# leagrieder/MultiMeditron

Measured on AMD Instinct MI355X. Metric: image-text samples/sec/node fwd+bwd, Llama-3.1-8B+ViT-L/14 bf16, higher is better.
Workload: dtype bf16; 1 GPU; llama31_8b_vitl14_s2048_b4; per_gpu_batch=4, global_batch=4, seq_len=2048, training_mode=FULL, parallelism=dp1

## Files before the change

include/mm_hip.h:

```cpp
#ifndef MM_HIP_H
#define MM_HIP_H

#include <stdint.h>

#ifdef __cplusplus
extern "C" {
#endif

typedef enum { MM_BF16 = 0, MM_F32 = 1 } mm_dtype;

enum { MM_OK = 0, MM_ERR_ARG = -1, MM_ERR_ALIGN = -2, MM_ERR_UNSUPPORTED = -3, MM_ERR_LAUNCH = -4 };

enum {
  MM_GEMM_NT = 0,
  MM_GEMM_NN = 1,
  MM_GEMM_TN = 2
};

enum {
  MM_EPI_BIAS = 1,
  MM_EPI_GELU_ERF = 2,
  MM_EPI_QUICK_GELU = 4,
  MM_EPI_RESIDUAL = 8,
  MM_EPI_ACCUMULATE = 16,
// ... 23 lines not shown

int mm_splice_build_map(const int64_t* batch_idx, const int64_t* token_range, int n_mod, int S, int T,
                        int32_t* src_map, void* stream);
int mm_embed_splice_fwd(int dtype, const void* emb, int64_t vocab, int H, const int64_t* ids, const void* proj,
                        const int32_t* src_map, int T, void* out, void* stream);
int mm_embed_sort_sizes(int T, int H, int64_t* order_elems, int64_t* scratch_floats);
int mm_embed_sort(const int64_t* ids, const int32_t* src_map, int T, int64_t vocab, int32_t* key_ws, int32_t* order,
                  int32_t* skey, void* stream);
int mm_embed_splice_bwd(int dtype, const void* dE, int H, const int64_t* ids, const int32_t* src_map, int T,
                        const int64_t* batch_idx, const int64_t* token_range, int n_mod, int S, void* dproj,
                        void* demb, int64_t vocab, const int32_t* order, const int32_t* skey, float* scratch,
                        int accumulate, void* stream);

int mm_patchify(int dtype, const float* pixels, int n, int himg, int wimg, int ps, int kpad, void* patches, void* stream);
int mm_vit_embed_fwd(int dtype, const void* patch_out, const void* cls, const void* pos, int n, int P, int D,
                     void* x, void* stream);
int mm_vit_embed_bwd(int dtype, const void* dx, int n, int P, int D, void* dpatch_out, void* dcls, void* dpos,
                     int accumulate, void* stream);
int mm_bcast_add(int dtype, const void* x, const void* b, int n, int64_t L, void* y, void* stream);
int mm_head_pad(int dtype, const void* src, int64_t rows, int nheads, int d, int dpad, void* dst, int inverse, void* stream);
int mm_drop_cls_fwd(int dtype, const void* src, int n, int P, int D, void* dst, void* stream);
int mm_drop_cls_bwd(int dtype, const void* ddst, int n, int P, int D, void* dsrc, void* stream);
int mm_rows_select(int dtype, const void* src, int64_t ld_src, const int* map, int n_src, int n_dst, int D, void* dst,
                   int64_t ld_dst, void* stream);

int mm_rmsnorm_fwd(int dtype, const void* x, const void* w, int M, int H, float eps, void* y, float* rstd, void* stream);
int mm_rmsnorm_bwd(int dtype, const void* dy, const void* x, const void* w, const float* rstd, int M, int H,
                   void* dx, float* dw_partial, const void* dres, void* stream);
int mm_layernorm_fwd(int dtype, const void* x, const void* w, const void* b, int M, int H, float eps, void* y,
                     float* mean, float* rstd, void* stream);
int mm_layernorm_bwd(int dtype, const void* dy, const void* x, const void* w, const float* mean, const float* rstd,
                     int M, int H, void* dx, float* dw_partial, float* db_partial, const void* dres, void* stream);
int mm_norm_bwd_blocks(int M);
int mm_reduce_partials(int dtype, const float* partial, int nblk, int H, void* out, int accumulate, void* stream);
int mm_reduce_partials2(int dtype, const float* partial0, const float* partial1, int nblk, int H, void* out0, void* out1, int accumulate0,
                        int accumulate1, void* stream);

int mm_rope_table(const int64_t* position_ids, const float* inv_freq, int T, int half, int round_bf16, float* cos_t,
                  float* sin_t, void* stream);
int mm_rope_apply(int dtype, void* x, int T, int nheads, int D, int ld, const float* cos_t, const float* sin_t,
                  int inverse, void* stream);

int mm_attn_fwd(int dtype, const void* q, const void* k, const void* v, int B, int Sq, int Skv, int Hq, int Hkv, int D,
                int64_t q_sb, int64_t q_ss, int64_t q_sh, int64_t k_sb, int64_t k_ss, int64_t k_sh, int64_t v_sb,
                int64_t v_ss, int64_t v_sh, const int64_t* key_mask, int causal, float scale, void* out, float* lse,
                void* stream);
int mm_attn_bwd(int dtype, const void* q, const void* k, const void* v, const void* out, const void* dout, const float* lse,
                int B, int Sq, int Skv, int Hq, int Hkv, int D, int64_t q_sb, int64_t q_ss, int64_t q_sh, int64_t k_sb,
                int64_t k_ss, int64_t k_sh, int64_t v_sb, int64_t v_ss, int64_t v_sh, const int64_t* key_mask, int causal,
                float scale, void* dq, void* dk, void* dv, float* delta, void* stream);

int mm_rope_append(int dtype, void* x, int T, int Hq, int Hkv, int D, int ld, const float* cos_t, const float* sin_t,
                   void* kdst, void* vdst, int64_t dstride, void* stream);

int mm_qk_norm_rope_fwd(int dtype, const void* x, int ld_in, int T, int Hq, int Hkv, int D, const void* w_q, const void* w_k, float eps,
                        const float* cos_t, const float* sin_t, void* out, int ld_out, float* rstd, void* stream);
int mm_qk_norm_bwd_blocks(int T);
int mm_qk_norm_rope_bwd(int dtype, const void* dqk, int ld_dqk, const void* x, int ld_x, int T, int Hq, int Hkv, int D, const void* w_q,
                        const void* w_k, const float* rstd, const float* cos_t, const float* sin_t, void* dx, int ld_dx, float* dwq_partial,
                        float* dwk_partial, void* stream);
int mm_qk_norm_rope_append(int dtype, void* x, int T, int Hq, int Hkv, int D, int ld, const void* w_q, const void* w_k, float eps,
                           const float* cos_t, const float* sin_t, void* kdst, void* vdst, int64_t dstride, void* stream);

int mm_decode_gateup_swiglu(int dtype, int M, int I, int K, const void* X, int ldx, const void* Wgu, int ldw, void* ACT, int ldact,
                            const void* in_norm_w, float eps, void* stream);
int mm_decode_qkv_rope_append(int dtype, int M, int Hq, int Hkv, int D, int K, const void* X, int ldx, const void* W, int ldw,
// ... 89 lines not shown
```

multimeditron_amd/csrc/mm_attn.hip:

```cpp
#include <string.h>

#include "mm_common.h"

namespace {

struct AttnArgs {
  const void *q, *k, *v;
  int B, Sq, Skv, Hq, Hkv;
  int64_t q_sb, q_ss, q_sh, k_sb, k_ss, k_sh, v_sb, v_ss, v_sh;
  const int64_t* kmask;
  int causal;
  float scale;
  void* out;
  float* lse;
  const void* dout;
  const float* delta;
  void *dq, *dk, *dv;
  int diag;
  int prio;
};

constexpr float LOG2E = 1.4426950408889634f;
constexpr float LN2 = 0.6931471805599453f;

template <int D> __device__ __forceinline__ int v_swz(int row) {
  if constexpr (D == 128) return (row & 3) << 1;
  else return ((row >> 1) & 1) << 1;
}

template <int D, int ROWS>
struct KcStage {
  static constexpr int NI = ROWS * (D / 8) / 256;
  u32x4 r[NI];
  __device__ __forceinline__ void load(const bf16* base, int64_t row_stride, int row0, int nrows_valid) {
    const int l = threadIdx.x & 63, w = threadIdx.x >> 6;
    constexpr int HALVES = D / 64;
#pragma unroll
    for (int i = 0; i < NI; ++i) {
      const int u = w * NI + i;
      const int rg = u / HALVES, dh = u % HALVES;
      const int row = rg * 8 + (l & 7), dc = dh * 8 + (l >> 3);
      u32x4 v = {0u, 0u, 0u, 0u};
      if (row0 + row < nrows_valid) v = *(const u32x4*)(base + (int64_t)(row0 + row) * row_stride + dc * 8);
      r[i] = v;
    }
  }
  __device__ __forceinline__ void store(char* tile) const {
    const int l = threadIdx.x & 63, w = threadIdx.x >> 6;
    constexpr int HALVES = D / 64;
#pragma unroll
// ... 193 lines not shown
    for (int db = 0; db < NDB; ++db)
#pragma unroll
      for (int rg = 0; rg < 4; ++rg) {
        bf16x4 o;
#pragma unroll
        for (int e = 0; e < 4; ++e) o[e] = (bf16)(o_acc[db][rg * 4 + e] * inv);
        *(bf16x4*)(orow + db * 32 + 8 * rg + 4 * h) = o;
      }
    if (h == 0) a.lse[((int64_t)b * a.Hq + hq) * a.Sq + qi] = l_tot > 0.f ? (m_run + log2f(l_tot)) * LN2 : INFINITY;
  }
}

template <typename T>
__global__ void attn_delta_kernel(const T* o, const T* dout, int B, int Sq, int Hq, int D, float* delta) {
  constexpr int VN = Vec16<T>::N;
  const int lpr = D / VN;
  const int64_t total = (int64_t)B * Sq * Hq;
  const int64_t tid = (int64_t)blockIdx.x * blockDim.x + threadIdx.x;
  const bool vec = (D % VN) == 0 && lpr <= 64 && (lpr & (lpr - 1)) == 0;
  if (!vec) {
    const int64_t wave = tid >> 6;
    const int lane = threadIdx.x & 63;
    if (wave >= total) return;
    float s = 0.f;
    for (int d = lane; d < D; d += 64) s += to_f32(o[wave * D + d]) * to_f32(dout[wave * D + d]);
    s = wave_sum(s);
    if (lane == 0) {
      const int hq = (int)(wave % Hq);
      const int64_t bs = wave / Hq;
      delta[((bs / Sq) * Hq + hq) * Sq + bs % Sq] = s;
    }
    return;
  }
  const int64_t row = tid / lpr;
  const int c = (int)(tid % lpr);
  float s = 0.f;
  if (row < total) {
    const Vec16<T> a = *(const Vec16<T>*)(o + row * D + c * VN), d = *(const Vec16<T>*)(dout + row * D + c * VN);
#pragma unroll
    for (int k = 0; k < VN; ++k) s += a.get(k) * d.get(k);
  }
  for (int off = lpr >> 1; off > 0; off >>= 1) s += __shfl_xor(s, off, 64);
  if (row < total && c == 0) {
    const int hq = (int)(row % Hq);
    const int64_t bs = row / Hq;
    delta[((bs / Sq) * Hq + hq) * Sq + bs % Sq] = s;
  }
}

template <int D>
__global__ __launch_bounds__(256, (D == 128 ? 1 : 2)) void attn_bwd_dq_kernel(AttnArgs a) {
  constexpr int BKV = 64, NDS = D / 16, NDB = D / 32;
  extern __shared__ __attribute__((aligned(16))) char smem[];
  char* Kc = smem;
  char* Vc = smem + BKV * D * 2;
  char* Kr = smem + 2 * BKV * D * 2;
  const int l = threadIdx.x & 63, w = threadIdx.x >> 6, h = l >> 5;
  const int b = blockIdx.z, hq = blockIdx.y, hkv = hq / (a.Hq / a.Hkv);
  const int q0 = blockIdx.x * 128 + w * 32;
  const int qi = q0 + (l & 31);
  const int shift = a.Skv - a.Sq;
  const bf16* Q = (const bf16*)a.q + b * a.q_sb + hq * a.q_sh;
  const bf16* K = (const bf16*)a.k + b * a.k_sb + hkv * a.k_sh;
  const bf16* V = (const bf16*)a.v + b * a.v_sb + hkv * a.v_sh;
  const bf16* dO = (const bf16*)a.dout + ((int64_t)b * a.Sq * a.Hq + hq) * D;

  bf16x8 qf[NDS], dof[NDS];
  {
    const bf16* qrow = qi < a.Sq ? Q + (int64_t)qi * a.q_ss : nullptr;
    const bf16* drow = qi < a.Sq ? dO + (int64_t)qi * a.Hq * D : nullptr;
#pragma unroll
    for (int ds = 0; ds < NDS; ++ds) {
      qf[ds] = row_frag_global(qrow, ds);
      dof[ds] = row_frag_global(drow, ds);
    }
  }
  const float sc = a.scale * LOG2E;
  float lse2 = INFINITY, dlt = 0.f;
  if (qi < a.Sq) {
// ... 978 lines not shown
  }
}

__global__ __launch_bounds__(512, 2) void attn_bwd_dq128p_kernel(AttnArgs a) {
  constexpr int BKV = 64, NDS = 8, NDB = 4, TILE = BKV * 256;
  extern __shared__ __attribute__((aligned(16))) char smem[];
  const int l = threadIdx.x & 63, h = l >> 5;
  const int w = __builtin_amdgcn_readfirstlane(threadIdx.x >> 6);
  int qblk, b, hq;
  attn_work_item(blockIdx.x, (a.Sq + 255) / 256, a.B, a.Hq, a.Hkv, a.causal != 0, qblk, b, hq);
  const int hkv = hq / (a.Hq / a.Hkv);
  const int q0 = qblk * 256 + w * 32;
  const int qi = q0 + (l & 31);
  const int shift = a.Skv - a.Sq;
  const bf16* Q = (const bf16*)a.q + b * a.q_sb + hq * a.q_sh;
  const bf16* dO = (const bf16*)a.dout + ((int64_t)b * a.Sq * a.Hq + hq) * 128;
  const SRsrc rk = rows_rsrc((const bf16*)a.k + b * a.k_sb + hkv * a.k_sh, a.Skv, a.k_ss);
  const SRsrc rv = rows_rsrc((const bf16*)a.v + b * a.v_sb + hkv * a.v_sh, a.Skv, a.v_ss);
  const unsigned lds0 = (unsigned)(uintptr_t)LDS_PTR(char, smem);
  const ImgaBases bases = imga_bases(smem, 0);

  bf16x8 qf[NDS], dof[NDS];
  {
    const bf16* qrow = qi < a.Sq ? Q + (int64_t)qi * a.q_ss : nullptr;
    const bf16* drow = qi < a.Sq ? dO + (int64_t)qi * a.Hq * 128 : nullptr;
#pragma unroll
    for (int ds = 0; ds < NDS; ++ds) {
      qf[ds] = row_frag_global(qrow, ds);
      dof[ds] = row_frag_global(drow, ds);
    }
  }
  const float sc = a.scale * LOG2E;
  float lse2 = INFINITY, dlt = 0.f;
  if (qi < a.Sq) {
    lse2 = a.lse[((int64_t)b * a.Hq + hq) * a.Sq + qi] * LOG2E;
    dlt = a.delta[((int64_t)b * a.Hq + hq) * a.Sq + qi];
  }
  f32x16 dq_acc[NDB];
#pragma unroll
  for (int i = 0; i < NDB; ++i)
#pragma unroll
    for (int r = 0; r < 16; ++r) dq_acc[i][r] = 0.f;

  int ntiles = (a.Skv + BKV - 1) / BKV;
  if (a.causal) {
    const int qmax = min(a.Sq - 1, qblk * 256 + 255) + shift;
    ntiles = qmax < 0 ? 0 : min(ntiles, qmax / BKV + 1);
  }
  unsigned lk[2], lv[2];
  imga_lane_patterns(lk, lv, a.k_ss, a.v_ss);
  constexpr int NST = 3;
  if (ntiles > 0) imga_issue_kv(w, lds0, 0, rk, rv, lk, lv, a.k_ss, a.v_ss, TILE);
  if (ntiles > 1) imga_issue_kv(w, lds0 + 2 * TILE, BKV, rk, rv, lk, lv, a.k_ss, a.v_ss, TILE);
  for (int t = 0; t < ntiles; ++t) {
    const int kv0 = t * BKV;
    if (t + 1 < ntiles) asm volatile("s_waitcnt vmcnt(8)" ::: "memory");
    else asm volatile("s_waitcnt vmcnt(0)" ::: "memory");
    __builtin_amdgcn_s_barrier();
    if (t + 2 < ntiles) imga_issue_kv(w, lds0 + (unsigned)(((t + 2) % NST) * 2 * TILE), (t + 2) * BKV, rk, rv, lk, lv, a.k_ss, a.v_ss, TILE);
    if (q0 >= a.Sq || (a.causal && kv0 > q0 + 31 + shift)) continue;
    const int so = (t % NST) * 2 * TILE;
    bool kvalid = (kv0 + l) < a.Skv;
    if (kvalid && a.kmask) kvalid = a.kmask[(int64_t)b * a.Skv + kv0 + l] != 0;
    const unsigned long long kbits = __ballot(kvalid);
    const bool need_mask = (kbits != ~0ull) || (a.causal && (kv0 + BKV - 1) > (q0 + shift));
    constexpr int RD = 4;
#pragma unroll 1
// ... 328 lines not shown
    for (int j = 0; j < 8; ++j) red_o[w][kq][g][row * 8 + j] = o[g][j];
  float lt = l_run + __shfl_xor(l_run, 16, 64);
  lt += __shfl_xor(lt, 32, 64);
  if (kq == 0 && row < G) { red_ml[w][row][0] = m_run; red_ml[w][row][1] = lt; }
  __syncthreads();
  for (int i = threadIdx.x; i < G * D; i += 256) {
    const int g = i / D, d = i % D;
    float mn = -INFINITY;
#pragma unroll
    for (int ww = 0; ww < 4; ++ww) mn = fmaxf(mn, red_ml[ww][g][0]);
    float ltot = 0.f, ot = 0.f;
#pragma unroll
    for (int ww = 0; ww < 4; ++ww) {
      const float al = mn == -INFINITY ? 0.f : __builtin_amdgcn_exp2f(red_ml[ww][g][0] - mn);
      ltot += red_ml[ww][g][1] * al;
      ot += ((red_o[ww][0][g][d] + red_o[ww][1][g][d]) + (red_o[ww][2][g][d] + red_o[ww][3][g][d])) * al;
    }
    float* rec = a.ws + (((int64_t)b * a.Hq + hkv * G + g) * a.nsplit + split) * (D + 2);
    rec[2 + d] = ot;
    if (d == 0) { rec[0] = mn; rec[1] = ltot; }
  }
}

template <int D>
__global__ void attn_decode_merge_kernel(const float* ws, int nsplit, bf16* out) {
  const int row = blockIdx.x, d = threadIdx.x;
  out[(int64_t)row * D + d] = decode_merge_one<D>(ws + (int64_t)row * nsplit * (D + 2), nsplit, d);
}

int g_attn_diag = 0;
int g_attn_q_prio = 1;
int g_attn_decode_mfma = 1;
int g_attn_decode_wgs = 768;

template <typename Kernel>
void launch128(Kernel kern, int64_t nwg, size_t lds, const AttnArgs& a, hipStream_t s) {
  (void)hipFuncSetAttribute((const void*)kern, hipFuncAttributeMaxDynamicSharedMemorySize, (int)lds);
  hipLaunchKernelGGL(kern, dim3((unsigned)nwg), dim3(512), lds, s, a);
}

template <int D>
int launch_bf16_fwd(const AttnArgs& a, hipStream_t s) {
  if constexpr (D == 128) {
    const int64_t nwg = (int64_t)((a.Sq + 255) / 256) * a.Hq * a.B;
    if (nwg > 0x7FFFFFFF) return MM_ERR_ARG;
    if (a.Skv <= 256 * 1024) launch128(attn_fwd128q_kernel<4, 4>, nwg, 4 * 2 * 64 * 256 + (size_t)((a.Skv + 63) / 64) * 8, a, s);
    else launch128(attn_fwd128p_kernel, nwg, 3 * 2 * 64 * 256, a, s);
  } else {
    const size_t lds = 2 * 64 * D * 2;
    dim3 grid((a.Sq + 127) / 128, a.Hq, a.B), block(256);
    hipLaunchKernelGGL(attn_fwd_kernel<D>, grid, block, lds, s, a);
  }
  return MM_OK;
}
template <int D>
int launch_bf16_bwd(const AttnArgs& a, hipStream_t s) {
  if constexpr (D == 128) {
    const int64_t nwg_q = (int64_t)((a.Sq + 255) / 256) * a.Hq * a.B;
    const int nkb = (a.Skv + 127) / 128;
    const int64_t nwg_kv = (int64_t)((nkb + 1) / 2) * a.Hkv * a.B;
    if (nwg_q > 0x7FFFFFFF || nwg_kv > 0x7FFFFFFF) return MM_ERR_ARG;
    launch128(attn_bwd_dq128p_kernel, nwg_q, 3 * 2 * 64 * 256, a, s);
    launch128(attn_bwd_dkv128_pairp_kernel<8, false>, nwg_kv, 2 * 128 * 256 + 8 * 32 * 256 + 4 * 64 * sizeof(float), a, s);
  } else {
    const size_t lds_dq = 3 * 64 * D * 2, lds_dkv = 4 * 32 * D * 2 + 64 * sizeof(float);
    hipLaunchKernelGGL(attn_bwd_dq_kernel<D>, dim3((a.Sq + 127) / 128, a.Hq, a.B), dim3(256), lds_dq, s, a);
    hipLaunchKernelGGL(attn_bwd_dkv_kernel<D>, dim3((a.Skv + 127) / 128, a.Hkv, a.B), dim3(256), lds_dkv, s, a);
  }
  return MM_OK;
}

}

int mm_attn_option(const char* name, int value) {
  if (!strcmp(name, "attn_decode_mfma")) { g_attn_decode_mfma = value != 0; return MM_OK; }
  if (!strcmp(name, "attn_decode_wgs")) { if (value < 1) return MM_ERR_ARG; g_attn_decode_wgs = value; return MM_OK; }
  if (!strcmp(name, "attn_q_prio")) { g_attn_q_prio = value; return MM_OK; }
  if (!strcmp(name, "attn_diag")) { g_attn_diag = value; return MM_OK; }
  return MM_ERR_ARG;
}

static int check_common(int dtype, int B, int Sq, int Skv, int Hq, int Hkv, int D) {
  if (B < 0 || Sq < 0 || Skv < 0 || Hq <= 0 || Hkv <= 0 || Hq % Hkv || D <= 0) return MM_ERR_ARG;
  if (dtype == MM_BF16 && D != 64 && D != 128) return MM_ERR_UNSUPPORTED;
  if (dtype == MM_F32 && (D > 256 || Skv > 12000)) return MM_ERR_UNSUPPORTED;
  if (dtype != MM_BF16 && dtype != MM_F32) return MM_ERR_UNSUPPORTED;
  return MM_OK;
}

extern "C" int mm_attn_fwd(int dtype, const void* q, const void* k, const void* v, int B, int Sq, int Skv, int Hq, int Hkv, int D,
                           int64_t q_sb, int64_t q_ss, int64_t q_sh, int64_t k_sb, int64_t k_ss, int64_t k_sh, int64_t v_sb, int64_t v_ss,
                           int64_t v_sh, const int64_t* key_mask, int causal, float scale, void* out, float* lse, void* stream) {
  int rc = check_common(dtype, B, Sq, Skv, Hq, Hkv, D);
  if (rc) return rc;
  if (!q || !k || !v || !out || !lse) return MM_ERR_ARG;
  if (B == 0 || Sq == 0) return MM_OK;
  AttnArgs a{};
  a.prio = g_attn_q_prio;
  a.diag = g_attn_diag;
  a.q = q; a.k = k; a.v = v; a.B = B; a.Sq = Sq; a.Skv = Skv; a.Hq = Hq; a.Hkv = Hkv;
  a.q_sb = q_sb; a.q_ss = q_ss; a.q_sh = q_sh; a.k_sb = k_sb; a.k_ss = k_ss; a.k_sh = k_sh; a.v_sb = v_sb; a.v_ss = v_ss; a.v_sh = v_sh;
  a.kmask = key_mask; a.causal = causal; a.scale = scale; a.out = out; a.lse = lse;
  hipStream_t s = (hipStream_t)stream;
  if (dtype == MM_BF16) {
    if ((q_sb | q_ss | q_sh | k_sb | k_ss | k_sh | v_sb | v_ss | v_sh) & 7) return MM_ERR_ALIGN;
    if (!mm_aligned16(q) || !mm_aligned16(k) || !mm_aligned16(v) || !mm_aligned16(out)) return MM_ERR_ALIGN;
    rc = D == 128 ? launch_bf16_fwd<128>(a, s) : launch_bf16_fwd<64>(a, s);
  } else {
    const size_t lds = (size_t)(Skv + D) * sizeof(float);
    hipLaunchKernelGGL(attn_fwd_f32_kernel, dim3(Sq, Hq, B), dim3(64), lds, s, a, D);
  }
  MM_CHECK_LAUNCH();
  return rc;
}

extern "C" int mm_attn_bwd(int dtype, const void* q, const void* k, const void* v, const void* out, const void* dout, const float* lse,
                           int B, int Sq, int Skv, int Hq, int Hkv, int D, int64_t q_sb, int64_t q_ss, int64_t q_sh, int64_t k_sb,
                           int64_t k_ss, int64_t k_sh, int64_t v_sb, int64_t v_ss, int64_t v_sh, const int64_t* key_mask, int causal,
                           float scale, void* dq, void* dk, void* dv, float* delta, void* stream) {
  int rc = check_common(dtype, B, Sq, Skv, Hq, Hkv, D);
  if (rc) return rc;
  if (!q || !k || !v || !out || !dout || !lse || !dq || !dk || !dv || !delta) return MM_ERR_ARG;
  if (B == 0 || Sq == 0) return MM_OK;
  AttnArgs a{};
  a.prio = g_attn_q_prio;
  a.diag = g_attn_diag;
  a.q = q; a.k = k; a.v = v; a.B = B; a.Sq = Sq; a.Skv = Skv; a.Hq = Hq; a.Hkv = Hkv;
  a.q_sb = q_sb; a.q_ss = q_ss; a.q_sh = q_sh; a.k_sb = k_sb; a.k_ss = k_ss; a.k_sh = k_sh; a.v_sb = v_sb; a.v_ss = v_ss; a.v_sh = v_sh;
  a.kmask = key_mask; a.causal = causal; a.scale = scale; a.out = (void*)out; a.lse = (float*)lse;
  a.dout = dout; a.delta = delta; a.dq = dq; a.dk = dk; a.dv = dv;
  hipStream_t s = (hipStream_t)stream;
  const int64_t rows = (int64_t)B * Sq * Hq;
  if (dtype == MM_BF16) {
    if ((q_sb | q_ss | q_sh | k_sb | k_ss | k_sh | v_sb | v_ss | v_sh) & 7) return MM_ERR_ALIGN;
    hipLaunchKernelGGL(attn_delta_kernel<bf16>, dim3((unsigned)((rows * (D / 8) + 255) / 256)), dim3(256), 0, s, (const bf16*)out, (const bf16*)dout, B, Sq, Hq, D, delta);
    rc = D == 128 ? launch_bf16_bwd<128>(a, s) : launch_bf16_bwd<64>(a, s);
  } else {
    {
      const int lpr = D / 4;
      const bool vec = (D % 4) == 0 && lpr <= 64 && (lpr & (lpr - 1)) == 0;
      const int64_t nthr = vec ? rows * lpr : rows * 64;
      hipLaunchKernelGGL(attn_delta_kernel<float>, dim3((unsigned)((nthr + 255) / 256)), dim3(256), 0, s, (const float*)out, (const float*)dout, B, Sq, Hq, D, delta);
    }
    const size_t lds = (size_t)(2 * Skv + 2 * D) * sizeof(float);
    hipLaunchKernelGGL(attn_bwd_f32_kernel, dim3(Sq, Hq, B), dim3(64), lds, s, a, D);
  }
  MM_CHECK_LAUNCH();
  return rc;
}

extern "C" int mm_attn_decode_splits(int B, int Hkv, int Skv) {
  if (B <= 0 || Hkv <= 0 || Skv <= 0) return 1;
  int n = (g_attn_decode_wgs + B * Hkv - 1) / (B * Hkv);
  const int cap = (Skv + 63) / 64;
  if (n > cap) n = cap;
  return n < 1 ? 1 : n;
}

extern "C" int mm_attn_decode(int dtype, const void* q, const void* k, const void* v, int B, int Skv, int Hq, int Hkv, int D,
                              int64_t q_sb, int64_t q_sh, int64_t k_sb, int64_t k_ss, int64_t k_sh, int64_t v_sb, int64_t v_ss,
                              int64_t v_sh, const int64_t* key_mask, float scale, void* out, float* workspace, int nsplit,
                              int* sync, void* stream) {
  if (B < 0 || Skv <= 0 || Hq <= 0 || Hkv <= 0 || Hq % Hkv || nsplit < 1) return MM_ERR_ARG;
  if (dtype != MM_BF16 || (D != 64 && D != 128)) return MM_ERR_UNSUPPORTED;
  const int G = Hq / Hkv;
  if (G != 1 && G != 2 && G != 4 && G != 7 && G != 8) return MM_ERR_UNSUPPORTED;
  if (!q || !k || !v || !out || !workspace) return MM_ERR_ARG;
  if (B == 0) return MM_OK;
  if ((q_sb | q_sh | k_sb | k_ss | k_sh | v_sb | v_ss | v_sh) & 7) return MM_ERR_ALIGN;
  if (!mm_aligned16(q) || !mm_aligned16(k) || !mm_aligned16(v)) return MM_ERR_ALIGN;
  DecodeArgs a{q, k, v, B, Skv, Hq, Hkv, q_sb, q_sh, k_sb, k_ss, k_sh, v_sb, v_ss, v_sh, key_mask, scale, out, workspace, nsplit, 0, sync};
  a.chunk = (Skv + nsplit - 1) / nsplit;
  hipStream_t s = (hipStream_t)stream;
  dim3 grid(nsplit, Hkv, B), block(256);
#define MM_DEC(DD, GG) hipLaunchKernelGGL((attn_decode_partial_kernel<DD, GG>), grid, block, 0, s, a)
#define MM_DEC_G(DD)                                                                                          \
// ... 19 lines not shown
```

multimeditron_amd/csrc/mm_rowwise.hip:

```cpp
#include "mm_common.h"

namespace {

constexpr int NORM_BWD_ROWS_PER_BLOCK = 16;

template <typename T, int CH>
__global__ __launch_bounds__(256) void rmsnorm_fwd_kernel(const T* x, const T* w, int M, int H, float eps, T* y, float* rstd) {
  __shared__ float red[8];
  constexpr int VN = Vec16<T>::N;
  const int row = blockIdx.x;
  const T* xr = x + (int64_t)row * H;
  T* yr = y + (int64_t)row * H;
  Vec16<T> xv[CH];
  float ss = 0.f;
#pragma unroll
  for (int c = 0; c < CH; ++c) {
    const int e = (c * 256 + threadIdx.x) * VN;
    if (e < H) {
      xv[c] = *(const Vec16<T>*)(xr + e);
#pragma unroll
      for (int i = 0; i < VN; ++i) { float f = xv[c].get(i); ss += f * f; }
    }
  }
  ss = block_sum_256(ss, red);
  const float rs = rsqrtf(ss / (float)H + eps);
  if (threadIdx.x == 0) rstd[row] = rs;
#pragma unroll
  for (int c = 0; c < CH; ++c) {
    const int e = (c * 256 + threadIdx.x) * VN;
    if (e < H) {
      Vec16<T> wv = *(const Vec16<T>*)(w + e), o;
#pragma unroll
// ... 22 lines not shown
  }
  const int r0 = blockIdx.x * NORM_BWD_ROWS_PER_BLOCK;
  const int r1 = min(M, r0 + NORM_BWD_ROWS_PER_BLOCK);
  for (int row = r0; row < r1; ++row) {
    const float rs = rstd[row];
    Vec16<T> xv[CH], gv[CH];
    float dot = 0.f;
#pragma unroll
    for (int c = 0; c < CH; ++c) {
      const int e = (c * 256 + threadIdx.x) * VN;
      if (e < H) {
        xv[c] = *(const Vec16<T>*)(x + (int64_t)row * H + e);
        gv[c] = *(const Vec16<T>*)(dy + (int64_t)row * H + e);
#pragma unroll
        for (int i = 0; i < VN; ++i) {
          const float xh = xv[c].get(i) * rs;
          const float g = gv[c].get(i);
          dw[c][i] += g * xh;
          dot += g * wv[c].get(i) * xh;
        }
      }
    }
    dot = block_sum_256(dot, red) / (float)H;
#pragma unroll
    for (int c = 0; c < CH; ++c) {
      const int e = (c * 256 + threadIdx.x) * VN;
      if (e < H) {
        Vec16<T> o, rv;
        if (dres) rv = *(const Vec16<T>*)(dres + (int64_t)row * H + e);
#pragma unroll
        for (int i = 0; i < VN; ++i) {
          const float xh = xv[c].get(i) * rs;
          o.set(i, rs * (gv[c].get(i) * wv[c].get(i) - xh * dot) + (dres ? rv.get(i) : 0.f));
        }
        *(Vec16<T>*)(dx + (int64_t)row * H + e) = o;
      }
    }
  }
#pragma unroll
  for (int c = 0; c < CH; ++c) {
    const int e = (c * 256 + threadIdx.x) * VN;
    if (e < H)
#pragma unroll
      for (int i = 0; i < VN; ++i) dwp[(int64_t)blockIdx.x * H + e + i] = dw[c][i];
  }
}

template <typename T, int CH>
__global__ __launch_bounds__(256) void layernorm_fwd_kernel(const T* x, const T* w, const T* b, int M, int H, float eps, T* y,
                                                            float* mean, float* rstd) {
  __shared__ float red[8];
  constexpr int VN = Vec16<T>::N;
  const int row = blockIdx.x;
  const T* xr = x + (int64_t)row * H;
  Vec16<T> xv[CH];
  float s = 0.f;
#pragma unroll
  for (int c = 0; c < CH; ++c) {
    const int e = (c * 256 + threadIdx.x) * VN;
    if (e < H) {
      xv[c] = *(const Vec16<T>*)(xr + e);
#pragma unroll
      for (int i = 0; i < VN; ++i) s += xv[c].get(i);
    }
  }
  const float mu = block_sum_256(s, red) / (float)H;
// ... 538 lines not shown
      Vec16<T> o;
#pragma unroll
      for (int k = 0; k < VN; ++k) o.set(k, acc[k]);
      *(Vec16<T>*)(out + (int64_t)b * L + c) = o;
    } else {
      for (int j = 0; j < J; ++j) {
        const Vec16<T> x = *(const Vec16<T>*)(X + ((int64_t)idx.v[j] * n + b) * L + c);
        Vec16<T> o;
#pragma unroll
        for (int k = 0; k < VN; ++k) o.set(k, w[j] * x.get(k));
        *(Vec16<T>*)(out + ((int64_t)b * J + j) * L + c) = o;
      }
    }
  } else {
    for (int j = 0; j < J; ++j) {
      const Vec16<T> d = *(const Vec16<T>*)(X + (mode == 0 ? (int64_t)b * L : ((int64_t)b * J + j) * L) + c);
      Vec16<T> o;
#pragma unroll
      for (int k = 0; k < VN; ++k) o.set(k, w[j] * d.get(k));
      *(Vec16<T>*)(out + ((int64_t)idx.v[j] * n + b) * L + c) = o;
    }
  }
}

template <typename S, typename D>
__global__ void cast_kernel(const S* s, D* d, int64_t n) {
  const int64_t i = (int64_t)blockIdx.x * blockDim.x + threadIdx.x;
  const int64_t stride = (int64_t)gridDim.x * blockDim.x;
  for (int64_t k = i; k < n; k += stride) d[k] = from_f32<D>(to_f32(s[k]));
}

template <typename T> inline int norm_ch(int H) { return (H + 256 * Vec16<T>::N - 1) / (256 * Vec16<T>::N); }

}

#define DISPATCH_CH(T, ch, ...)                            \
  switch (ch) {                                            \
    case 1: { constexpr int CH = 1; __VA_ARGS__; } break;  \
    case 2: { constexpr int CH = 2; __VA_ARGS__; } break;  \
    case 3: case 4: { constexpr int CH = 4; __VA_ARGS__; } break; \
    case 5: case 6: case 7: case 8: { constexpr int CH = 8; __VA_ARGS__; } break; \
    default: return MM_ERR_UNSUPPORTED;                    \
  }

extern "C" int mm_norm_bwd_blocks(int M) { return (M + NORM_BWD_ROWS_PER_BLOCK - 1) / NORM_BWD_ROWS_PER_BLOCK; }

extern "C" int mm_rmsnorm_fwd(int dtype, const void* x, const void* w, int M, int H, float eps, void* y, float* rstd, void* stream) {
  if (!x || !w || !y || !rstd || M < 0 || H <= 0) return MM_ERR_ARG;
  if (M == 0) return MM_OK;
  hipStream_t s = (hipStream_t)stream;
  if (dtype == MM_BF16) {
    if (H % 8) return MM_ERR_ALIGN;
    DISPATCH_CH(bf16, norm_ch<bf16>(H), hipLaunchKernelGGL((rmsnorm_fwd_kernel<bf16, CH>), dim3(M), dim3(256), 0, s, (const bf16*)x, (const bf16*)w, M, H, eps, (bf16*)y, rstd));
  } else {
    if (H % 4) return MM_ERR_ALIGN;
    DISPATCH_CH(float, norm_ch<float>(H), hipLaunchKernelGGL((rmsnorm_fwd_kernel<float, CH>), dim3(M), dim3(256), 0, s, (const float*)x, (const float*)w, M, H, eps, (float*)y, rstd));
  }
  MM_CHECK_LAUNCH();
  return MM_OK;
}

extern "C" int mm_rmsnorm_bwd(int dtype, const void* dy, const void* x, const void* w, const float* rstd, int M, int H, void* dx,
                              float* dwp, const void* dres, void* stream) {
  if (!dy || !x || !w || !rstd || !dx || !dwp || M < 0 || H <= 0) return MM_ERR_ARG;
  if (M == 0) return MM_OK;
  hipStream_t s = (hipStream_t)stream;
  const int nb = mm_norm_bwd_blocks(M);
  if (dtype == MM_BF16) {
    if (H % 8) return MM_ERR_ALIGN;
    DISPATCH_CH(bf16, norm_ch<bf16>(H), hipLaunchKernelGGL((rmsnorm_bwd_kernel<bf16, CH>), dim3(nb), dim3(256), 0, s, (const bf16*)dy, (const bf16*)x, (const bf16*)w, rstd, M, H, (bf16*)dx, dwp, (const bf16*)dres));
  } else {
    if (H % 4) return MM_ERR_ALIGN;
    DISPATCH_CH(float, norm_ch<float>(H), hipLaunchKernelGGL((rmsnorm_bwd_kernel<float, CH>), dim3(nb), dim3(256), 0, s, (const float*)dy, (const float*)x, (const float*)w, rstd, M, H, (float*)dx, dwp, (const float*)dres));
  }
  MM_CHECK_LAUNCH();
  return MM_OK;
}

extern "C" int mm_layernorm_fwd(int dtype, const void* x, const void* w, const void* b, int M, int H, float eps, void* y,
                                float* mean, float* rstd, void* stream) {
  if (!x || !w || !b || !y || !mean || !rstd || M < 0 || H <= 0) return MM_ERR_ARG;
  if (M == 0) return MM_OK;
  hipStream_t s = (hipStream_t)stream;
  if (dtype == MM_BF16) {
    if (H % 8) return MM_ERR_ALIGN;
    DISPATCH_CH(bf16, norm_ch<bf16>(H), hipLaunchKernelGGL((layernorm_fwd_kernel<bf16, CH>), dim3(M), dim3(256), 0, s, (const bf16*)x, (const bf16*)w, (const bf16*)b, M, H, eps, (bf16*)y, mean, rstd));
  } else {
    if (H % 4) return MM_ERR_ALIGN;
    DISPATCH_CH(float, norm_ch<float>(H), hipLaunchKernelGGL((layernorm_fwd_kernel<float, CH>), dim3(M), dim3(256), 0, s, (const float*)x, (const float*)w, (const float*)b, M, H, eps, (float*)y, mean, rstd));
  }
  MM_CHECK_LAUNCH();
  return MM_OK;
}

extern "C" int mm_layernorm_bwd(int dtype, const void* dy, const void* x, const void* w, const float* mean, const float* rstd,
                                int M, int H, void* dx, float* dwp, float* dbp, const void* dres, void* stream) {
  if (!dy || !x || !w || !mean || !rstd || !dx || !dwp || !dbp || M < 0 || H <= 0) return MM_ERR_ARG;
  if (M == 0) return MM_OK;
  hipStream_t s = (hipStream_t)stream;
  const int nb = mm_norm_bwd_blocks(M);
  if (dtype == MM_BF16) {
    if (H % 8) return MM_ERR_ALIGN;
    DISPATCH_CH(bf16, norm_ch<bf16>(H), hipLaunchKernelGGL((layernorm_bwd_kernel<bf16, CH>), dim3(nb), dim3(256), 0, s, (const bf16*)dy, (const bf16*)x, (const bf16*)w, mean, rstd, M, H, (bf16*)dx, dwp, dbp, (const bf16*)dres));
  } else {
    if (H % 4) return MM_ERR_ALIGN;
    DISPATCH_CH(float, norm_ch<float>(H), hipLaunchKernelGGL((layernorm_bwd_kernel<float, CH>), dim3(nb), dim3(256), 0, s, (const float*)dy, (const float*)x, (const float*)w, mean, rstd, M, H, (float*)dx, dwp, dbp, (const float*)dres));
// ... 307 lines not shown
```

multimeditron_amd/kernels.py:

```python
from __future__ import annotations

import math
from typing import Optional, Tuple

import torch

from . import _lib
from ._lib import (EPI_ACCUMULATE, EPI_BIAS, EPI_GELU_ERF, EPI_QUICK_GELU, EPI_RESIDUAL, GEMM_NN, GEMM_NT, GEMM_TN,
                   MM_BF16, MM_F32, call)

_DT = {torch.bfloat16: MM_BF16, torch.float32: MM_F32}


def dt(t: torch.Tensor) -> int:
    try:
        return _DT[t.dtype]
    except KeyError:
        raise TypeError(f"libmmhip supports bf16/f32 tensors, got {t.dtype}") from None


def _stream() -> int:
    return torch.cuda.current_stream().cuda_stream


# ... 270 lines not shown
    n, T, D = x.shape
    out = torch.empty((n, T - 1, D), dtype=x.dtype, device=x.device)
    call("mm_drop_cls_fwd", dt(x), _p(x), n, T - 1, D, _p(out), _stream())
    return out


def drop_cls_bwd(dy):
    n, P, D = dy.shape
    out = torch.empty((n, P + 1, D), dtype=dy.dtype, device=dy.device)
    call("mm_drop_cls_bwd", dt(dy), _p(dy), n, P, D, _p(out), _stream())
    return out


def rows_select(src2d, row_map, n_dst):
    D = src2d.shape[1]
    assert row_map.dtype == torch.int32 and row_map.is_contiguous() and row_map.numel() >= n_dst and src2d.stride(1) == 1
    out = torch.empty((n_dst, D), dtype=src2d.dtype, device=src2d.device)
    call("mm_rows_select", dt(src2d), _p(src2d), src2d.stride(0), _p(row_map), src2d.shape[0], n_dst, D, _p(out), D, _stream())
    return out


def rmsnorm_fwd(x2d, w, eps):
    M, H = x2d.shape
    y = torch.empty_like(x2d)
    rstd = torch.empty(M, dtype=torch.float32, device=x2d.device)
    call("mm_rmsnorm_fwd", dt(x2d), _p(x2d), _p(w), M, H, float(eps), _p(y), _p(rstd), _stream())
    return y, rstd


def norm_bwd_blocks(M):
    return _lib.lib().mm_norm_bwd_blocks(M)


def rmsnorm_bwd(dy2d, x2d, w, rstd, dres=None):
    M, H = x2d.shape
    dx = torch.empty_like(x2d)
    dwp = torch.empty((norm_bwd_blocks(M), H), dtype=torch.float32, device=x2d.device)
    call("mm_rmsnorm_bwd", dt(x2d), _p(dy2d), _p(x2d), _p(w), _p(rstd), M, H, _p(dx), _p(dwp), _p(dres), _stream())
    return dx, dwp


def layernorm_fwd(x2d, w, b, eps):
    M, H = x2d.shape
    y = torch.empty_like(x2d)
    mean = torch.empty(M, dtype=torch.float32, device=x2d.device)
    rstd = torch.empty(M, dtype=torch.float32, device=x2d.device)
    call("mm_layernorm_fwd", dt(x2d), _p(x2d), _p(w), _p(b), M, H, float(eps), _p(y), _p(mean), _p(rstd), _stream())
    return y, mean, rstd


def layernorm_bwd(dy2d, x2d, w, mean, rstd, dres=None):
    M, H = x2d.shape
    dx = torch.empty_like(x2d)
    nb = norm_bwd_blocks(M)
    dwp = torch.empty((nb, H), dtype=torch.float32, device=x2d.device)
    dbp = torch.empty((nb, H), dtype=torch.float32, device=x2d.device)
    call("mm_layernorm_bwd", dt(x2d), _p(dy2d), _p(x2d), _p(w), _p(mean), _p(rstd), M, H, _p(dx), _p(dwp), _p(dbp), _p(dres), _stream())
    return dx, dwp, dbp


def reduce_partials2(partial0, partial1, out0, out1, accumulate0, accumulate1):
    assert partial0.shape == partial1.shape and out0.dtype == out1.dtype
    call("mm_reduce_partials2", dt(out0), _p(partial0), _p(partial1), partial0.shape[0], partial0.shape[1], _p(out0), _p(out1), int(accumulate0),
         int(accumulate1), _stream())


def reduce_partials(partial, out, accumulate):
# ... 360 lines not shown
```

Before: 11.58 samples/s.

## Fold attention delta into dQ backward kernel and pipeline RMSNorm backward loads

For head dim 128, the softmax-backward delta (rowsum of O·dO) is now computed inside the dQ backward kernel from the O and dO fragments it already loads. The kernel also writes delta out for the other backward kernels, which removes a separate delta kernel launch. The standalone delta kernel becomes a grid-stride loop with 4-way unrolled loads and a capped grid. A new RMSNorm backward kernel prefetches the next row's x, dy and residual into registers while the current row is being reduced, and it is on by default. These changes trade extra register pressure for fewer launches and better latency hiding. They also rely on the other backward kernels reading delta only after the dQ kernel has written it.

```diff
diff --git a/include/mm_hip.h b/include/mm_hip.h
--- a/include/mm_hip.h
+++ b/include/mm_hip.h
@@ -79,6 +79,7 @@
 int mm_layernorm_bwd(int dtype, const void* dy, const void* x, const void* w, const float* mean, const float* rstd,
                      int M, int H, void* dx, float* dw_partial, float* db_partial, const void* dres, void* stream);
 int mm_norm_bwd_blocks(int M);
+int mm_rowwise_option(const char* name, int value);
 int mm_reduce_partials(int dtype, const float* partial, int nblk, int H, void* out, int accumulate, void* stream);
 int mm_reduce_partials2(int dtype, const float* partial0, const float* partial1, int nblk, int H, void* out0, void* out1, int accumulate0,
                         int accumulate1, void* stream);
diff --git a/multimeditron_amd/csrc/mm_attn.hip b/multimeditron_amd/csrc/mm_attn.hip
--- a/multimeditron_amd/csrc/mm_attn.hip
+++ b/multimeditron_amd/csrc/mm_attn.hip
@@ -14,8 +14,9 @@
   void* out;
   float* lse;
   const void* dout;
-  const float* delta;
+  float* delta;
   void *dq, *dk, *dv;
+  int delta_fold;
   int diag;
   int prio;
 };
@@ -275,19 +276,41 @@
     }
     return;
   }
-  const int64_t row = tid / lpr;
-  const int c = (int)(tid % lpr);
-  float s = 0.f;
-  if (row < total) {
-    const Vec16<T> a = *(const Vec16<T>*)(o + row * D + c * VN), d = *(const Vec16<T>*)(dout + row * D + c * VN);
-#pragma unroll
-    for (int k = 0; k < VN; ++k) s += a.get(k) * d.get(k);
-  }
-  for (int off = lpr >> 1; off > 0; off >>= 1) s += __shfl_xor(s, off, 64);
-  if (row < total && c == 0) {
-    const int hq = (int)(row % Hq);
-    const int64_t bs = row / Hq;
-    delta[((bs / Sq) * Hq + hq) * Sq + bs % Sq] = s;
+  constexpr int U = 4;
+  const int64_t nthr = (int64_t)gridDim.x * blockDim.x, nwork = total * lpr;
+  const int lsh = __builtin_ctz(lpr), c = (int)(tid & (lpr - 1));
+  for (int64_t t0 = tid; (t0 & ~(int64_t)63) < nwork; t0 += U * nthr) {
+    Vec16<T> av[U], dv[U];
+#pragma unroll
+    for (int u = 0; u < U; ++u) {
+      const int64_t row = (t0 + u * nthr) >> lsh;
+      if (row < total) {
+        av[u] = *(const Vec16<T>*)(o + row * D + c * VN);
+        dv[u] = *(const Vec16<T>*)(dout + row * D + c * VN);
+      }
+    }
+#pragma unroll
+    for (int u = 0; u < U; ++u) {
+      const int64_t row = (t0 + u * nthr) >> lsh;
+      float s = 0.f;
+      if (row < total) {
+#pragma unroll
+        for (int k = 0; k < VN; ++k) s = __fadd_rn(s, __fmul_rn(av[u].get(k), dv[u].get(k)));
+      }
+      for (int off = lpr >> 1; off > 0; off >>= 1) s += __shfl_xor(s, off, 64);
+      if (row < total && c == 0) {
+        int64_t at;
+        if (total <= 0x7FFFFFFF) {
+          const unsigned r = (unsigned)row, hq = r % (unsigned)Hq, bs = r / (unsigned)Hq;
+          at = ((int64_t)(bs / (unsigned)Sq) * Hq + hq) * Sq + bs % (unsigned)Sq;
+        } else {
+          const int hq = (int)(row % Hq);
+          const int64_t bs = row / Hq;
+          at = ((bs / Sq) * Hq + hq) * Sq + bs % Sq;
+        }
+        delta[at] = s;
+      }
+    }
   }
 }
 
@@ -1332,7 +1355,24 @@
   }
   const float sc = a.scale * LOG2E;
   float lse2 = INFINITY, dlt = 0.f;
-  if (qi < a.Sq) {
+  if (a.delta_fold) {
+    const bf16* orow = qi < a.Sq ? (const bf16*)a.out + (((int64_t)b * a.Sq + qi) * a.Hq + hq) * 128 : nullptr;
+    float sp[NDS];
+#pragma unroll
+    for (int ds = 0; ds < NDS; ++ds) {
+      const bf16x8 of = row_frag_global(orow, ds);
+      float t = 0.f;
+#pragma unroll
+      for (int k = 0; k < 8; ++k) t = __fadd_rn(t, __fmul_rn((float)of[k], (float)dof[ds][k]));
+      sp[ds] = t;
+    }
+    const float half_sum = ((sp[0] + sp[4]) + (sp[2] + sp[6])) + ((sp[1] + sp[5]) + (sp[3] + sp[7]));
+    dlt = half_sum + __shfl_xor(half_sum, 32, 64);
+    if (qi < a.Sq) {
+      lse2 = a.lse[((int64_t)b * a.Hq + hq) * a.Sq + qi] * LOG2E;
+      if (h == 0) a.delta[((int64_t)b * a.Hq + hq) * a.Sq + qi] = dlt;
+    }
+  } else if (qi < a.Sq) {
     lse2 = a.lse[((int64_t)b * a.Hq + hq) * a.Sq + qi] * LOG2E;
     dlt = a.delta[((int64_t)b * a.Hq + hq) * a.Sq + qi];
   }
@@ -1727,6 +1767,7 @@
 int g_attn_q_prio = 1;
 int g_attn_decode_mfma = 1;
 int g_attn_decode_wgs = 768;
+int g_attn_delta_fold = 1;
 
 template <typename Kernel>
 void launch128(Kernel kern, int64_t nwg, size_t lds, const AttnArgs& a, hipStream_t s) {
@@ -1772,6 +1813,7 @@
   if (!strcmp(name, "attn_decode_wgs")) { if (value < 1) return MM_ERR_ARG; g_attn_decode_wgs = value; return MM_OK; }
   if (!strcmp(name, "attn_q_prio")) { g_attn_q_prio = value; return MM_OK; }
   if (!strcmp(name, "attn_diag")) { g_attn_diag = value; return MM_OK; }
+  if (!strcmp(name, "attn_delta_fold")) { g_attn_delta_fold = value != 0; return MM_OK; }
   return MM_ERR_ARG;
 }
 
@@ -1809,6 +1851,17 @@
   return rc;
 }
 
+template <typename T>
+static void launch_delta(const void* out, const void* dout, int B, int Sq, int Hq, int D, float* delta, hipStream_t s) {
+  constexpr int VN = Vec16<T>::N;
+  const int64_t rows = (int64_t)B * Sq * Hq;
+  const int lpr = D / VN;
+  const bool vec = (D % VN) == 0 && lpr <= 64 && (lpr & (lpr - 1)) == 0;
+  int64_t nblk = ((vec ? rows * lpr : rows * 64) + 255) / 256;
+  if (vec && nblk > 4096) nblk = 4096;
+  hipLaunchKernelGGL(attn_delta_kernel<T>, dim3((unsigned)nblk), dim3(256), 0, s, (const T*)out, (const T*)dout, B, Sq, Hq, D, delta);
+}
+
 extern "C" int mm_attn_bwd(int dtype, const void* q, const void* k, const void* v, const void* out, const void* dout, const float* lse,
                            int B, int Sq, int Skv, int Hq, int Hkv, int D, int64_t q_sb, int64_t q_ss, int64_t q_sh, int64_t k_sb,
                            int64_t k_ss, int64_t k_sh, int64_t v_sb, int64_t v_ss, int64_t v_sh, const int64_t* key_mask, int causal,
@@ -1825,18 +1878,13 @@
   a.kmask = key_mask; a.causal = causal; a.scale = scale; a.out = (void*)out; a.lse = (float*)lse;
   a.dout = dout; a.delta = delta; a.dq = dq; a.dk = dk; a.dv = dv;
   hipStream_t s = (hipStream_t)stream;
-  const int64_t rows = (int64_t)B * Sq * Hq;
   if (dtype == MM_BF16) {
     if ((q_sb | q_ss | q_sh | k_sb | k_ss | k_sh | v_sb | v_ss | v_sh) & 7) return MM_ERR_ALIGN;
-    hipLaunchKernelGGL(attn_delta_kernel<bf16>, dim3((unsigned)((rows * (D / 8) + 255) / 256)), dim3(256), 0, s, (const bf16*)out, (const bf16*)dout, B, Sq, Hq, D, delta);
+    a.delta_fold = D == 128 && g_attn_delta_fold;
+    if (!a.delta_fold) launch_delta<bf16>(out, dout, B, Sq, Hq, D, delta, s);
     rc = D == 128 ? launch_bf16_bwd<128>(a, s) : launch_bf16_bwd<64>(a, s);
   } else {
-    {
-      const int lpr = D / 4;
-      const bool vec = (D % 4) == 0 && lpr <= 64 && (lpr & (lpr - 1)) == 0;
-      const int64_t nthr = vec ? rows * lpr : rows * 64;
-      hipLaunchKernelGGL(attn_delta_kernel<float>, dim3((unsigned)((nthr + 255) / 256)), dim3(256), 0, s, (const float*)out, (const float*)dout, B, Sq, Hq, D, delta);
-    }
+    launch_delta<float>(out, dout, B, Sq, Hq, D, delta, s);
     const size_t lds = (size_t)(2 * Skv + 2 * D) * sizeof(float);
     hipLaunchKernelGGL(attn_bwd_f32_kernel, dim3(Sq, Hq, B), dim3(64), lds, s, a, D);
   }
diff --git a/multimeditron_amd/csrc/mm_rowwise.hip b/multimeditron_amd/csrc/mm_rowwise.hip
--- a/multimeditron_amd/csrc/mm_rowwise.hip
+++ b/multimeditron_amd/csrc/mm_rowwise.hip
@@ -1,3 +1,5 @@
+#include <string.h>
+
 #include "mm_common.h"
 
 namespace {
@@ -86,6 +88,82 @@
         for (int i = 0; i < VN; ++i) {
           const float xh = xv[c].get(i) * rs;
           o.set(i, rs * (gv[c].get(i) * wv[c].get(i) - xh * dot) + (dres ? rv.get(i) : 0.f));
+        }
+        *(Vec16<T>*)(dx + (int64_t)row * H + e) = o;
+      }
+    }
+  }
+#pragma unroll
+  for (int c = 0; c < CH; ++c) {
+    const int e = (c * 256 + threadIdx.x) * VN;
+    if (e < H)
+#pragma unroll
+      for (int i = 0; i < VN; ++i) dwp[(int64_t)blockIdx.x * H + e + i] = dw[c][i];
+  }
+}
+
+template <typename T, int CH>
+__global__ __launch_bounds__(256) void rmsnorm_bwd_pipe_kernel(const T* dy, const T* x, const T* w, const float* rstd, int M, int H,
+                                                               T* dx, float* dwp, const T* dres) {
+  __shared__ float red[8];
+  constexpr int VN = Vec16<T>::N;
+  float dw[CH][VN];
+  Vec16<T> wv[CH];
+#pragma unroll
+  for (int c = 0; c < CH; ++c) {
+    const int e = (c * 256 + threadIdx.x) * VN;
+    if (e < H) wv[c] = *(const Vec16<T>*)(w + e);
+#pragma unroll
+    for (int i = 0; i < VN; ++i) dw[c][i] = 0.f;
+  }
+  const int r0 = blockIdx.x * NORM_BWD_ROWS_PER_BLOCK;
+  const int r1 = min(M, r0 + NORM_BWD_ROWS_PER_BLOCK);
+  Vec16<T> xn[CH] = {}, gn[CH] = {}, rn[CH] = {};
+  float rsn = 0.f;
+  auto request = [&](int row) {
+    rsn = rstd[row];
+#pragma unroll
+    for (int c = 0; c < CH; ++c) {
+      const int e = (c * 256 + threadIdx.x) * VN;
+      if (e < H) {
+        xn[c] = *(const Vec16<T>*)(x + (int64_t)row * H + e);
+        gn[c] = *(const Vec16<T>*)(dy + (int64_t)row * H + e);
+        if (dres) rn[c] = *(const Vec16<T>*)(dres + (int64_t)row * H + e);
+      }
+    }
+  };
+  if (r0 < r1) request(r0);
+  for (int row = r0; row < r1; ++row) {
+    const float rs = rsn;
+    Vec16<T> xv[CH], gv[CH], rv[CH];
+    float dot = 0.f;
+#pragma unroll
+    for (int c = 0; c < CH; ++c) {
+      const int e = (c * 256 + threadIdx.x) * VN;
+      if (e < H) {
+        xv[c] = xn[c];
+        gv[c] = gn[c];
+        rv[c] = rn[c];
+#pragma unroll
+        for (int i = 0; i < VN; ++i) {
+          const float xh = xv[c].get(i) * rs;
+          const float g = gv[c].get(i);
+          dw[c][i] += g * xh;
+          dot += g * wv[c].get(i) * xh;
+        }
+      }
+    }
+    if (row + 1 < r1) request(row + 1);
+    dot = block_sum_256(dot, red) / (float)H;
+#pragma unroll
+    for (int c = 0; c < CH; ++c) {
+      const int e = (c * 256 + threadIdx.x) * VN;
+      if (e < H) {
+        Vec16<T> o;
+#pragma unroll
+        for (int i = 0; i < VN; ++i) {
+          const float xh = xv[c].get(i) * rs;
+          o.set(i, rs * (gv[c].get(i) * wv[c].get(i) - xh * dot) + (dres ? rv[c].get(i) : 0.f));
         }
         *(Vec16<T>*)(dx + (int64_t)row * H + e) = o;
       }
@@ -690,6 +768,8 @@
 
 template <typename T> inline int norm_ch(int H) { return (H + 256 * Vec16<T>::N - 1) / (256 * Vec16<T>::N); }
 
+int g_rmsnorm_bwd_pipe = 1;
+
 }
 
 #define DISPATCH_CH(T, ch, ...)                            \
@@ -700,6 +780,12 @@
     case 5: case 6: case 7: case 8: { constexpr int CH = 8; __VA_ARGS__; } break; \
     default: return MM_ERR_UNSUPPORTED;                    \
   }
+
+extern "C" int mm_rowwise_option(const char* name, int value) {
+  if (!name) return MM_ERR_ARG;
+  if (!strcmp(name, "rmsnorm_bwd_pipe")) { g_rmsnorm_bwd_pipe = value != 0; return MM_OK; }
+  return MM_ERR_ARG;
+}
 
 extern "C" int mm_norm_bwd_blocks(int M) { return (M + NORM_BWD_ROWS_PER_BLOCK - 1) / NORM_BWD_ROWS_PER_BLOCK; }
 
@@ -726,10 +812,18 @@
   const int nb = mm_norm_bwd_blocks(M);
   if (dtype == MM_BF16) {
     if (H % 8) return MM_ERR_ALIGN;
-    DISPATCH_CH(bf16, norm_ch<bf16>(H), hipLaunchKernelGGL((rmsnorm_bwd_kernel<bf16, CH>), dim3(nb), dim3(256), 0, s, (const bf16*)dy, (const bf16*)x, (const bf16*)w, rstd, M, H, (bf16*)dx, dwp, (const bf16*)dres));
+    if (g_rmsnorm_bwd_pipe) {
+      DISPATCH_CH(bf16, norm_ch<bf16>(H), hipLaunchKernelGGL((rmsnorm_bwd_pipe_kernel<bf16, CH>), dim3(nb), dim3(256), 0, s, (const bf16*)dy, (const bf16*)x, (const bf16*)w, rstd, M, H, (bf16*)dx, dwp, (const bf16*)dres));
+    } else {
+      DISPATCH_CH(bf16, norm_ch<bf16>(H), hipLaunchKernelGGL((rmsnorm_bwd_kernel<bf16, CH>), dim3(nb), dim3(256), 0, s, (const bf16*)dy, (const bf16*)x, (const bf16*)w, rstd, M, H, (bf16*)dx, dwp, (const bf16*)dres));
+    }
   } else {
     if (H % 4) return MM_ERR_ALIGN;
-    DISPATCH_CH(float, norm_ch<float>(H), hipLaunchKernelGGL((rmsnorm_bwd_kernel<float, CH>), dim3(nb), dim3(256), 0, s, (const float*)dy, (const float*)x, (const float*)w, rstd, M, H, (float*)dx, dwp, (const float*)dres));
+    if (g_rmsnorm_bwd_pipe) {
+      DISPATCH_CH(float, norm_ch<float>(H), hipLaunchKernelGGL((rmsnorm_bwd_pipe_kernel<float, CH>), dim3(nb), dim3(256), 0, s, (const float*)dy, (const float*)x, (const float*)w, rstd, M, H, (float*)dx, dwp, (const float*)dres));
+    } else {
+      DISPATCH_CH(float, norm_ch<float>(H), hipLaunchKernelGGL((rmsnorm_bwd_kernel<float, CH>), dim3(nb), dim3(256), 0, s, (const float*)dy, (const float*)x, (const float*)w, rstd, M, H, (float*)dx, dwp, (const float*)dres));
+    }
   }
   MM_CHECK_LAUNCH();
   return MM_OK;
diff --git a/multimeditron_amd/kernels.py b/multimeditron_amd/kernels.py
--- a/multimeditron_amd/kernels.py
+++ b/multimeditron_amd/kernels.py
@@ -326,7 +326,22 @@
     return _lib.lib().mm_norm_bwd_blocks(M)
 
 
+_rmsnorm_bwd_pipe = None
+
+
+def _apply_rmsnorm_bwd_pipe():
+    global _rmsnorm_bwd_pipe
+    want = _os.environ.get("MM_RMSNORM_BWD_PIPE")
+    if want is None and _rmsnorm_bwd_pipe is None:
+        return
+    want = int(want != "0")
+    if want != _rmsnorm_bwd_pipe:
+        call("mm_rowwise_option", b"rmsnorm_bwd_pipe", want)
+        _rmsnorm_bwd_pipe = want
+
+
 def rmsnorm_bwd(dy2d, x2d, w, rstd, dres=None):
+    _apply_rmsnorm_bwd_pipe()
     M, H = x2d.shape
     dx = torch.empty_like(x2d)
     dwp = torch.empty((norm_bwd_blocks(M), H), dtype=torch.float32, device=x2d.device)
```

After: 11.61 samples/s, median of 4. No clear change (+0.3%).
